# Coloquinte/sleekit

Measured on AMD Instinct MI355X. Metric: Mweights/sec quantized (GPTQ 3-bit, 4096x4096 layer), higher is better.
Workload: dtype f64; 1 GPU; 8 layers 4096x4096, 8-level uniform codebook (GPTQ 3-bit), act_order=diag, damp=0.01, local-search moves=0, layer error included; distinct_inputs=8, allocator_settle_steps=15, gpu_max_hw_queues=4

## Files before the change

sleekit_amd/csrc/api.hip:

```cpp
#include "mfma32.h"
#include "mfma64.h"

namespace slk {

__global__ __launch_bounds__(256) void k_probe_f64(double *sink, int iters) {
    double4_t c0 = {0, 0, 0, 0}, c1 = c0, c2 = c0, c3 = c0;
    const double a = 1.0 + threadIdx.x * 1e-3, b = 1.0 - threadIdx.x * 1e-3;
    for (int i = 0; i < iters; ++i) {
        c0 = __builtin_amdgcn_mfma_f64_16x16x4f64(a, b, c0, 0, 0, 0);
        c1 = __builtin_amdgcn_mfma_f64_16x16x4f64(b, a, c1, 0, 0, 0);
        c2 = __builtin_amdgcn_mfma_f64_16x16x4f64(a, a, c2, 0, 0, 0);
        c3 = __builtin_amdgcn_mfma_f64_16x16x4f64(b, b, c3, 0, 0, 0);
    }
    const double4_t s = c0 + c1 + c2 + c3;
    if (s[0] + s[1] + s[2] + s[3] == 12345.678) sink[0] = s[0];
}

template <int NACC>
__global__ __launch_bounds__(256) void k_probe_f64_n(double *sink, int iters) {
    double4_t c[NACC];
    double a[NACC], b[NACC];
#pragma unroll
    for (int i = 0; i < NACC; ++i) {
        c[i] = (double4_t){0, 0, 0, 0};
// ... 67 lines not shown
}

using namespace slk;

extern "C" {

int slk_probe_chain(double *out, int iters, int mode, slk_stream_t stream) {
    SLK_REQUIRE(out && iters > 0, "bad arguments");
    hipStream_t s = as_stream(stream);
    SLK_RUN("probe_chain", 0, 0, s, k_probe_chain<<<1, 64, 0, s>>>(out, iters, mode));
    return SLK_OK;
}

size_t slk_workspace_bytes(int R, int n) {
    if (R < 0 || n <= 0) return 0;
    const size_t ld = (size_t)slk_factor_ld(n);
    const size_t rn = (size_t)(R > 0 ? R : 1) * (size_t)n;
    size_t factor = 2 * ld * ld * sizeof(double) + 2 * (ld / 64) * sizeof(int);
    size_t loop = 2 * rn * sizeof(float) + (size_t)n * sizeof(int) + 64 * sizeof(float) + 5 * 256;
    size_t search = rn * sizeof(float) + (size_t)(R + n) * sizeof(float) + (size_t)R * ((n + 127) / 128) * sizeof(float) + 4096;
    size_t error = 6 * (rn + 128 * (size_t)n) + 6 * (size_t)n * n + 4 * (size_t)R * ((n + 127) / 128) * sizeof(float) + 8192;
    size_t prep = 64 * sizeof(float) + (size_t)n * (sizeof(double) + 1);
    search += error;
    size_t m = factor;
    if (loop > m) m = loop;
    if (search > m) m = search;
    if (error > m) m = error;
    if (prep > m) m = prep;
    return m + (1u << 16);
}

size_t slk_workspace_bytes_batch(int batch, int rows_per_layer, int n) {
    if (batch < 1 || batch > 64 || rows_per_layer < 0 || n <= 0 || (long long)batch * rows_per_layer > 0x7fffffffLL) return 0;
    return slk_workspace_bytes(batch * rows_per_layer, n) + (size_t)(batch - 1) * 6 * (size_t)n * n +
           (size_t)batch * n * (sizeof(int) + sizeof(float)) + (size_t)(batch - 1) * 64 * sizeof(float) +
           4096;
}

int slk_probe_mfma_f64(double *sink, int blocks, int iters, slk_stream_t stream) {
    SLK_REQUIRE(sink && blocks > 0 && iters > 0, "bad arguments");
    hipStream_t s = as_stream(stream);
    SLK_RUN("probe_mfma_f64", 4.0 * 2048 * 4 * iters * blocks, 0, s, k_probe_f64<<<blocks, 256, 0, s>>>(sink, iters));
    return SLK_OK;
}

int slk_probe_mfma_f64_acc(double *sink, int blocks, int iters, int nacc, slk_stream_t stream) {
    SLK_REQUIRE(sink && blocks > 0 && iters > 0 && (nacc == 1 || nacc == 2 || nacc == 4 || nacc == 8 || nacc == 16), "bad arguments");
    hipStream_t s = as_stream(stream);
    if (nacc == 1)
        SLK_RUN("probe_mfma_f64", 1.0 * 2048 * 4 * iters * blocks, 0, s, k_probe_f64_n<1><<<blocks, 256, 0, s>>>(sink, iters));
    else if (nacc == 2)
        SLK_RUN("probe_mfma_f64", 2.0 * 2048 * 4 * iters * blocks, 0, s, k_probe_f64_n<2><<<blocks, 256, 0, s>>>(sink, iters));
    else if (nacc == 4)
        SLK_RUN("probe_mfma_f64", 4.0 * 2048 * 4 * iters * blocks, 0, s, k_probe_f64_n<4><<<blocks, 256, 0, s>>>(sink, iters));
    else if (nacc == 8)
        SLK_RUN("probe_mfma_f64", 8.0 * 2048 * 4 * iters * blocks, 0, s, k_probe_f64_n<8><<<blocks, 256, 0, s>>>(sink, iters));
    else
        SLK_RUN("probe_mfma_f64", 16.0 * 2048 * 4 * iters * blocks, 0, s, k_probe_f64_n<16><<<blocks, 256, 0, s>>>(sink, iters));
    return SLK_OK;
}

int slk_probe_mfma_f32(float *sink, int blocks, int iters, slk_stream_t stream) {
    SLK_REQUIRE(sink && blocks > 0 && iters > 0, "bad arguments");
    hipStream_t s = as_stream(stream);
    SLK_RUN("probe_mfma_f32", 4.0 * 4096 * 4 * iters * blocks, 0, s, k_probe_f32<<<blocks, 256, 0, s>>>(sink, iters));
    return SLK_OK;
}

}

#include <atomic>
#include <map>
#include <mutex>
#include <string>
#include <vector>
#include <strings.h>

namespace slk {
namespace {
const char *const kOptNames[OPT_COUNT] = {
    "NO_FAST_LEAF", "NO_DEFER", "NO_WINDOW2", "WIN_DBG", "NO_REGULAR_SEARCH", "NO_FAST_SEARCH_DIV",
    "NO_ERROR_SPLITK", "ERROR_CB", "NO_SYM_ERROR", "NO_BF16_ERROR", "NO_BF16_DMA", "NO_BF16_HESSIAN",
    "ERROR_F32_BELOW", "NO_BF16_ASYM", "NO_SYM_AVERAGE", "NO_WAVE_SEARCH", "LOOKAHEAD", "WINDOW_ROWS", "PANEL_SPLIT", "ROWS_BELOW_WIDE",
    "NO_LOOP_ERROR",
};
std::atomic<int> g_opts[OPT_COUNT];
std::once_flag g_opts_once;
void opts_from_env() {
    for (int i = 0; i < OPT_COUNT; ++i) {
        const std::string name = std::string("SLK_") + kOptNames[i];
        const char *v = getenv(name.c_str());
        int val = 0;
        if (v) {
            val = atoi(v);
            if (val == 0 && v[0] != '0') val = 1;
        }
        g_opts[i].store(val, std::memory_order_relaxed);
    }
}
int opt_index(const char *name) {
    if (!name) return -1;
    if (strncasecmp(name, "SLK_", 4) == 0) name += 4;
    for (int i = 0; i < OPT_COUNT; ++i)
        if (strcasecmp(name, kOptNames[i]) == 0) return i;
    return -1;
}
std::mutex g_lds_mu;
std::map<std::pair<const void *, int>, size_t> g_lds_set;
}

int opt(Opt o) {
    std::call_once(g_opts_once, opts_from_env);
    return g_opts[o].load(std::memory_order_relaxed);
}

namespace {
std::mutex g_helper_mu;
struct HelperRec {
    Helper h;
    int made;
};
std::map<std::pair<int, hipStream_t>, HelperRec> g_helpers;
}

hipError_t helper_for(hipStream_t main, int need, Helper *out) {
    if (need > HELPER_EVENTS) return hipErrorInvalidValue;
    int device = 0;
    hipError_t e = hipGetDevice(&device);
    if (e != hipSuccess) return e;
    std::lock_guard<std::mutex> lock(g_helper_mu);
    auto it = g_helpers.find({device, main});
    if (it == g_helpers.end()) {
        HelperRec r{};
        e = hipStreamCreateWithFlags(&r.h.stream, hipStreamNonBlocking);
        if (e != hipSuccess) return e;
        e = hipStreamCreateWithFlags(&r.h.stream2, hipStreamNonBlocking);
        if (e != hipSuccess) {
            (void)hipStreamDestroy(r.h.stream);
            return e;
        }
        r.h.events = new hipEvent_t[HELPER_EVENTS]();
        r.made = 0;
        it = g_helpers.emplace(std::make_pair(device, main), r).first;
    }
    HelperRec &r = it->second;
    const int had = r.made;
    while (r.made < need) {
        e = hipEventCreateWithFlags(&r.h.events[r.made], hipEventDisableTiming);
        if (e != hipSuccess) {
            while (r.made > had) (void)hipEventDestroy(r.h.events[--r.made]);
            if (had == 0) {
                (void)hipStreamDestroy(r.h.stream);
                (void)hipStreamDestroy(r.h.stream2);
                delete[] r.h.events;
                g_helpers.erase(it);
            }
            return e;
        }
        ++r.made;
    }
    *out = r.h;
    return hipSuccess;
}

static hipError_t release_helpers() {
    std::lock_guard<std::mutex> lock(g_helper_mu);
    hipError_t first = hipSuccess;
// ... 156 lines not shown
```

sleekit_amd/csrc/common.h:

```cpp
#pragma once

#include <hip/hip_runtime.h>
#include <stddef.h>
#include <stdint.h>
#include <stdio.h>

#include "../../include/sleekit_amd.h"

namespace slk {

void set_error(const char *fmt, ...);

#define SLK_REQUIRE(cond, ...)          \
    do {                                \
        if (!(cond)) {                  \
            slk::set_error(__VA_ARGS__); \
            return SLK_E_ARG;           \
        }                               \
    } while (0)

#define SLK_HIP(call)                                                                  \
    do {                                                                               \
        hipError_t e_ = (call);                                                        \
        if (e_ != hipSuccess) {                                                        \
            slk::set_error("%s failed: %s (%s:%d)", #call, hipGetErrorString(e_), __FILE__, __LINE__); \
            return SLK_E_HIP;                                                          \
        }                                                                              \
    } while (0)

#define SLK_LAUNCH_CHECK() SLK_HIP(hipGetLastError())

struct ProfScope {
    int slot;
    hipStream_t stream;
    ProfScope(const char *name, double flops, double bytes, hipStream_t s);
    ~ProfScope();
};

void prof_next_width(long workgroups);

#define SLK_RUN(name, flops, bytes, stream, ...)                 \
    do {                                                         \
        {                                                        \
            slk::ProfScope prof_scope_(name, flops, bytes, stream); \
            __VA_ARGS__;                                         \
        }                                                        \
        SLK_LAUNCH_CHECK();                                      \
    } while (0)

#define SLK_RUN_W(name, flops, bytes, wgs, stream, ...) \
    do {                                                \
        slk::prof_next_width((long)(wgs));              \
        SLK_RUN(name, flops, bytes, stream, __VA_ARGS__); \
    } while (0)

enum Opt {
    OPT_NO_FAST_LEAF,
    OPT_NO_DEFER,
    OPT_NO_WINDOW2,
    OPT_WIN_DBG,
    OPT_NO_REGULAR_SEARCH,
    OPT_NO_FAST_SEARCH_DIV,
    OPT_NO_ERROR_SPLITK,
    OPT_ERROR_CB,
    OPT_NO_SYM_ERROR,
    OPT_NO_BF16_ERROR,
    OPT_NO_BF16_DMA,
    OPT_NO_BF16_HESSIAN,
    OPT_ERROR_F32_BELOW,
    OPT_NO_BF16_ASYM,
    OPT_NO_SYM_AVERAGE,
    OPT_NO_WAVE_SEARCH,
    OPT_LOOKAHEAD,
    OPT_WINDOW_ROWS,
    OPT_PANEL_SPLIT,
    OPT_ROWS_BELOW_WIDE,
    OPT_NO_LOOP_ERROR,
    OPT_COUNT
};
int opt(Opt o);

struct Helper {
    hipStream_t stream;
    hipStream_t stream2;
    hipEvent_t *events;
};
constexpr int HELPER_EVENTS = 512;
hipError_t helper_for(hipStream_t main, int need, Helper *out);

hipError_t lds_opt_in(const void *kernel, size_t bytes);
#define SLK_LDS_OPT_IN(kernel, bytes) SLK_HIP(slk::lds_opt_in(reinterpret_cast<const void *>(kernel), (bytes)))

struct PtrTable {
    const float *p[64];
};

constexpr int LOOP_LAYERS = 16;
struct LayerTable {
    const float *W[LOOP_LAYERS], *scale[LOOP_LAYERS];
    const long long *order[LOOP_LAYERS];
    const double *U[LOOP_LAYERS];
};
template <class T>
__device__ __forceinline__ const T *layer_base(const T *const (&column)[LOOP_LAYERS], int b, size_t stride) {
    return column[b % LOOP_LAYERS] + (size_t)(b - b % LOOP_LAYERS) * stride;
}

int row_errors_products(const float *W, const float *Q, const float *const *Hs, int batch, int rpl, int n, const int *sym_known,
                        float *row_err, float *G, void *workspace, size_t ws_bytes, slk_stream_t stream);

int loop_error_means(const float *const *Hs, int batch, int n, float *out, hipStream_t s);

static inline hipStream_t as_stream(slk_stream_t s) { return reinterpret_cast<hipStream_t>(s); }

static inline size_t align_up(size_t x, size_t a) { return (x + a - 1) / a * a; }

struct Arena {
    char *base;
    size_t size, used;
    Arena(void *p, size_t bytes) : base(static_cast<char *>(p)), size(bytes), used(0) {}
    template <class T>
    T *take(size_t count) {
        size_t off = align_up(used, 256);
        size_t end = off + count * sizeof(T);
        if (end > size || base == nullptr) return nullptr;
        used = end;
        return reinterpret_cast<T *>(base + off);
    }
};

struct Grid {
    float zero, step, top;
    const float *table;
    int n;
};

static inline Grid make_grid(int levels, double lo, double hi, const float *table = nullptr) {
    Grid g;
    g.zero = (float)lo;
    g.step = (float)((hi - lo) / (double)(levels - 1));
    g.top = (float)(levels - 1);
    g.table = table;
    g.n = levels;
    return g;
}

__device__ __forceinline__ float grid_pos(float x, const Grid g, float shift, float first, float last) {
    float t = (x - g.zero) / g.step;
    t = t + shift;
    t = rintf(t);
    return fminf(fmaxf(t, first), last);
}
__device__ __forceinline__ float grid_val(float t, const Grid g) { return t * g.step + g.zero; }
__device__ __forceinline__ float grid_value(float x, const Grid g) {
    return grid_val(grid_pos(x, g, 0.0f, 0.0f, g.top), g);
}

__device__ __forceinline__ int table_index(float x, const Grid g) {
    const float *lim = g.table + g.n;
    int lo = 0, hi = g.n - 1;
// ... 106 lines not shown
```

sleekit_amd/csrc/factor.hip:

```cpp
#include <stdlib.h>

#include "mfma64.h"

namespace slk {

constexpr int PANEL = 64;
constexpr int OUTER_SMALL = 256, OUTER_LARGE = 512;
constexpr int LOOKAHEAD_MIN_TILES = 24;

__device__ long long g_panel_cycles[16];

constexpr int TP = 66;

struct PanelSmem {
    double t[PANEL][TP];
    double x[PANEL][TP];
    double a21[PANEL][TP];
    double lb[PANEL][TP];
    double rdiag[PANEL];
    int early_count;
};

#ifndef NEWTON_STEPS
#define NEWTON_STEPS 2
// ... 314 lines not shown
            acc, ts, kprev, kprev + PANEL, [&](int k, double(&v)[8]) { load8d<true>(pa + k, v); },
            [&](int k, double(&v)[8]) { load8d<true>(pb + k, v); });
        tile64_foreach2(old, acc, [&](int r, int c, double o, double v) { pc[(size_t)r * ld + c] = o - v; });
        return;
    }
    BelowSmem &sm = *reinterpret_cast<BelowSmem *>(smem_raw);
    X += (size_t)blockIdx.z * ld * ld;
    const int lane = t & 63, wave = t >> 6;
    const bool has_prev = kprev >= 0;
    const int sr = t >> 2, sc8 = (t & 3) * 16;
    const int first = (int)blockIdx.x * per_wg, last = min(first + per_wg, tiles_below);
    double vt[16], vb[16];
    auto fetch_tile = [&](int rt) {
        const int r0 = k0 + PANEL * (rt + 1);
        const double *pt = A + (size_t)(r0 + sr) * ld + k0 + sc8;
        load8d<true>(pt, *reinterpret_cast<double(*)[8]>(&vt[0]));
        load8d<true>(pt + 8, *reinterpret_cast<double(*)[8]>(&vt[8]));
        if (has_prev) {
            const double *pl = A + (size_t)(r0 + sr) * ld + kprev + sc8;
            load8d<true>(pl, *reinterpret_cast<double(*)[8]>(&vb[0]));
            load8d<true>(pl + 8, *reinterpret_cast<double(*)[8]>(&vb[8]));
        }
    };
    {
        double vx[16], vk[16];
        const double *px = X + (size_t)(k0 + sr) * ld + k0 + sc8;
        load8d<true>(px, *reinterpret_cast<double(*)[8]>(&vx[0]));
        load8d<true>(px + 8, *reinterpret_cast<double(*)[8]>(&vx[8]));
        if (has_prev) {
            const double *pk = A + (size_t)(k0 + sr) * ld + kprev + sc8;
            load8d<true>(pk, *reinterpret_cast<double(*)[8]>(&vk[0]));
            load8d<true>(pk + 8, *reinterpret_cast<double(*)[8]>(&vk[8]));
        }
        fetch_tile(first);
#pragma unroll
        for (int e = 0; e < 16; e += 2) {
            *reinterpret_cast<double2_t *>(&sm.x[sr][sc8 + e]) = (double2_t){vx[e], vx[e + 1]};
            if (has_prev) *reinterpret_cast<double2_t *>(&sm.lk[sr][sc8 + e]) = (double2_t){vk[e], vk[e + 1]};
        }
    }
    for (int rt = first; rt < last; ++rt) {
        const int r0 = k0 + PANEL * (rt + 1);
#pragma unroll
        for (int e = 0; e < 16; e += 2) {
            *reinterpret_cast<double2_t *>(&sm.a21[sr][sc8 + e]) = (double2_t){vt[e], vt[e + 1]};
            if (has_prev) *reinterpret_cast<double2_t *>(&sm.lb[sr][sc8 + e]) = (double2_t){vb[e], vb[e + 1]};
        }
        __syncthreads();
        if (rt + 1 < last) fetch_tile(rt + 1);
        if (has_prev) {
#pragma unroll
            for (int cb = 0; cb < 4; ++cb) {
                double4_t acc = {0.0, 0.0, 0.0, 0.0};
#pragma unroll
                for (int kq = 0; kq < 4; ++kq) acc = blk_mma_abt(&sm.lb[16 * wave][16 * kq], &sm.lk[16 * cb][16 * kq], acc, 1.0, lane);
                double *cp = &sm.a21[16 * wave][16 * cb];
                double4_t o = blk_load_d(cp, lane);
#pragma unroll
                for (int r = 0; r < 4; ++r) o[r] = o[r] - acc[r];
                blk_store_d(cp, lane, o);
            }
            asm volatile("s_waitcnt lgkmcnt(0)" ::: "memory");
        }
#pragma unroll
        for (int cb = 0; cb < 4; ++cb) {
            double4_t acc = {0.0, 0.0, 0.0, 0.0};
#pragma unroll
            for (int k = 0; k < 4; ++k)
                if (k <= cb) acc = blk_mma_abt(&sm.a21[16 * wave][16 * k], &sm.x[16 * cb][16 * k], acc, 1.0, lane);
#pragma unroll
            for (int r = 0; r < 4; ++r) A[(size_t)(r0 + 16 * wave + (lane >> 4) + 4 * r) * ld + k0 + 16 * cb + (lane & 15)] = acc[r];
        }
        if (rt + 1 < last) __syncthreads();
    }
}


constexpr int INFO_HANDOFF_TIMEOUT = 0x7fffffff;
constexpr bool slk_chain_addressable(int ld) { return (size_t)ld * (size_t)ld * sizeof(double) <= 0xffffffffull; }

typedef unsigned int u32x4_t __attribute__((ext_vector_type(4)));
typedef unsigned int u32x2_t __attribute__((ext_vector_type(2)));
constexpr int AUX_SC1 = 16;

struct GBuf {
    __amdgpu_buffer_rsrc_t rs;
    __device__ __forceinline__ GBuf(const double *base, size_t bytes)
        : rs(__builtin_amdgcn_make_buffer_rsrc(const_cast<double *>(base), 0, (int)(bytes > 0xffffffffull ? 0xffffffffull : bytes), 0x00020000)) {}
    template <int AUX>
    __device__ __forceinline__ double2_t load2(unsigned elem) const {
        const u32x4_t v = __builtin_amdgcn_raw_buffer_load_b128(rs, elem * 8u, 0, AUX);
        return (double2_t){__hiloint2double((int)v[1], (int)v[0]), __hiloint2double((int)v[3], (int)v[2])};
    }
    template <int AUX>
    __device__ __forceinline__ void store2(unsigned elem, double2_t x) const {
        const u32x4_t v = {(unsigned)__double2loint(x[0]), (unsigned)__double2hiint(x[0]), (unsigned)__double2loint(x[1]), (unsigned)__double2hiint(x[1])};
        __builtin_amdgcn_raw_buffer_store_b128(v, rs, elem * 8u, 0, AUX);
    }
};

__device__ __forceinline__ int flag_peek(const int *p) { return __hip_atomic_load(p, __ATOMIC_RELAXED, __HIP_MEMORY_SCOPE_AGENT); }
__device__ __forceinline__ bool flag_wait(const int *p, int want) {
    bool ok = flag_peek(p) >= want;
    if (!ok) {
        const unsigned long long t0 = __builtin_amdgcn_s_memrealtime();
        for (;;) {
            __builtin_amdgcn_s_sleep(1);
            if (flag_peek(p) >= want) {
                ok = true;
                break;
            }
            if (__builtin_amdgcn_s_memrealtime() - t0 > 200000000ull) break;
        }
    }
    __builtin_amdgcn_fence(__ATOMIC_ACQUIRE, "wavefront");
    return ok;
}
__device__ __forceinline__ void flag_publish(int *p, int value) {
    asm volatile("s_waitcnt vmcnt(0)" ::: "memory");
    __syncthreads();
    if (threadIdx.x == 0) __hip_atomic_store(p, value, __ATOMIC_RELAXED, __HIP_MEMORY_SCOPE_AGENT);
}

struct TileRegs {
    double2_t v[8];
};
template <int AUX, int J0 = 0, int J1 = 8>
__device__ __forceinline__ void tile_fetch(TileRegs &r, const GBuf &g, unsigned elem0, int ld) {
    const int t = threadIdx.x;
#pragma unroll
    for (int j = J0; j < J1; ++j) r.v[j] = g.load2<AUX>(elem0 + (unsigned)(8 * j + (t >> 5)) * (unsigned)ld + 2u * (t & 31));
}
template <int J0 = 0, int J1 = 8>
__device__ __forceinline__ void tile_stash(double (*img)[TP], const TileRegs &r) {
    const int t = threadIdx.x;
#pragma unroll
    for (int j = J0; j < J1; ++j) *reinterpret_cast<double2_t *>(&img[8 * j + (t >> 5)][2 * (t & 31)]) = r.v[j];
}
template <int AUX, int J0 = 0, int J1 = 8>
__device__ __forceinline__ void tile_store_from_lds(const GBuf &g, unsigned elem0, int ld, const double (*img)[TP]) {
    const int t = threadIdx.x;
#pragma unroll
    for (int j = J0; j < J1; ++j)
        g.store2<AUX>(elem0 + (unsigned)(8 * j + (t >> 5)) * (unsigned)ld + 2u * (t & 31), *reinterpret_cast<const double2_t *>(&img[8 * j + (t >> 5)][2 * (t & 31)]));
}

template <class Early>
__device__ __forceinline__ int diag_tile_factor(PanelSmem &sm, int lane, int wave, Early rows_0_and_1_are_in) {
    auto diag_inverse = [&](int kb) {
        const int c0 = 16 * kb, c = lane & 15;
        double xv[16];
#pragma unroll
        for (int i = 0; i < 16; ++i) {
            double s = 0.0;
#pragma unroll
            for (int u = 0; u < i; ++u) s = __builtin_fma(sm.t[c0 + i][c0 + u], xv[u], s);
            xv[i] = ((c == i ? 1.0 : 0.0) - s) * sm.rdiag[c0 + i];
        }
        if (lane < 16) {
#pragma unroll
            for (int i = 0; i < 16; ++i) sm.x[c0 + i][c0 + c] = xv[i];
        }
    };
    auto block_owner = [](int rb, int cb) { return cb == 1 ? rb : (rb == 3 && cb == 2 ? 2 : 1); };
    auto block_update = [&](int rb, int cb, int kb) {
        double *c = &sm.t[16 * rb][16 * cb];
        blk_store_d(c, lane, blk_mma_abt(&sm.t[16 * rb][16 * kb], &sm.t[16 * cb][16 * kb], blk_load_d(c, lane), -1.0, lane));
    };
    auto x_inner = [&](int rb, int cb) {
        double4_t sacc = {0.0, 0.0, 0.0, 0.0};
#pragma unroll
        for (int k = 0; k < 4; ++k)
            if (k >= cb && k < rb) sacc = blk_mma_ab(&sm.t[16 * rb][16 * k], &sm.x[16 * k][16 * cb], sacc, lane);
        return sacc;
    };
    auto x_finish = [&](int rb, int cb, double4_t sacc) {
        const double4_t z = {0.0, 0.0, 0.0, 0.0};
        blk_store_d(&sm.x[16 * rb][16 * cb], lane, blk_mma_a_reg(&sm.x[16 * rb][16 * rb], sacc, z, -1.0, lane));
    };
    auto x_block = [&](int rb, int cb) { x_finish(rb, cb, x_inner(rb, cb)); };
    auto own_writes = [&]() { asm volatile("s_waitcnt lgkmcnt(0)" ::: "memory"); };
    int first_bad = PANEL;
#pragma unroll
    for (int kb = 0; kb < 4; ++kb) {
        const int c0 = 16 * kb;
        if (wave == 0) {
            const int row = c0 + lane;
            const bool live = row < PANEL;
            double a[16];
#pragma unroll
            for (int c = 0; c < 16; ++c) a[c] = live ? sm.t[live ? row : 0][c0 + c] : 0.0;
#pragma unroll
            for (int j = 0; j < 16; ++j) {
                double piv = readlane_f64(a[j], j);
                const bool bad = !(piv > 0.0);
                first_bad = (bad && first_bad == PANEL) ? c0 + j : first_bad;
                piv = bad ? 1.0 : piv;
                const double r = rsqrt_newton(piv);
                const double lj = a[j] * r;
                a[j] = lj;
                sm.rdiag[c0 + j] = r;
#pragma unroll
                for (int c = j + 1; c < 16; ++c) a[c] = __builtin_fma(-lj, readlane_f64(lj, c), a[c]);
            }
            if (live) {
#pragma unroll
                for (int c = 0; c < 16; ++c) sm.t[row][c0 + c] = (c0 + c <= row) ? a[c] : 0.0;
            }
        } else if (kb == 0) {
        } else if (wave == 3) {
            diag_inverse(kb - 1);
            own_writes();
            if (kb == 2) x_block(1, 0);
            if (kb == 3) {
                x_block(2, 1);
                x_block(2, 0);
            }
        } else {
#pragma unroll
            for (int rb = kb + 1; rb < 4; ++rb)
#pragma unroll
                for (int cb = kb + 1; cb <= rb; ++cb)
                    if (block_owner(rb, cb) == wave) block_update(rb, cb, kb - 1);
            if (kb == 3) rows_0_and_1_are_in(wave - 1);
        }
        __syncthreads();
        if (kb < 3) {
#pragma unroll
            for (int rb = kb + 1; rb < 4; ++rb)
                if (block_owner(rb, kb + 1) == wave) block_update(rb, kb + 1, kb);
            __syncthreads();
        }
    }
    double4_t row3 = {0.0, 0.0, 0.0, 0.0};
    if (wave == 3) diag_inverse(3);
    else row3 = x_inner(3, wave);
    __syncthreads();
    if (wave < 3) x_finish(3, wave, row3);
    __syncthreads();
    return first_bad;
}

template <bool BELOW>
__global__ __launch_bounds__(256) void k_chol_chain(double *__restrict__ Aall, int ld, int K0, int nb, double *__restrict__ Xall,
                                                    int *__restrict__ info, int *__restrict__ flags_all, int dbg) {
    extern __shared__ __attribute__((aligned(16))) char smem_raw[];
    PanelSmem &sm = *reinterpret_cast<PanelSmem *>(smem_raw);
    const int t = threadIdx.x, lane = t & 63, wave = t >> 6;
    const int r = BELOW ? nb + (int)blockIdx.x : (int)blockIdx.x, nt = ld / PANEL, p0 = K0 / PANEL;
    const int rq = BELOW ? nb : r;
    const size_t mat = (size_t)ld * ld;
    double *A = Aall + (size_t)blockIdx.z * mat;
    const GBuf ga(A, mat * sizeof(double)), gx(Xall + (size_t)blockIdx.z * mat, mat * sizeof(double));
    info += blockIdx.z;
    int *xready = flags_all + (size_t)blockIdx.z * 2 * nt, *rowdone = xready + nt;
    const int row0 = K0 + PANEL * r;
    auto elem = [&](int tr, int tc) { return (unsigned)(K0 + PANEL * tr) * (unsigned)ld + (unsigned)(K0 + PANEL * tc); };
    bool alive = true;
    if (t == 0) sm.early_count = 0;
    const bool timing = !BELOW && dbg && r > 0 && blockIdx.z == 0 && wave == 0;
    long long tmark = 0;
    auto lap = [&](int slot) {
        if (timing) {
            const long long now = (long long)__builtin_readcyclecounter();
            if (lane == 0 && slot >= 0) atomicAdd(reinterpret_cast<unsigned long long *>(&g_panel_cycles[slot]), (unsigned long long)(now - tmark));
            tmark = now;
        }
    };

    double4_t tp[3];
    if constexpr (!BELOW) {
        int i = 0;
#pragma unroll
        for (int rb = 0; rb < 4; ++rb)
#pragma unroll
            for (int cb = 0; cb <= rb; ++cb, ++i)
                if ((i & 3) == wave) {
#pragma unroll
                    for (int j = 0; j < 4; ++j) {
                        const int rr = 16 * rb + (lane >> 4) + 4 * j, cc = 16 * cb + (lane & 15);
                        tp[i >> 2][j] = (r > 0 || cc <= rr) ? A[(size_t)(row0 + rr) * ld + row0 + cc] : 0.0;
                    }
                }
    }
    auto update_cn = [&](double4_t(&cn)[4]) {
#pragma unroll
        for (int cb = 0; cb < 4; ++cb) {
            double4_t acc = {0.0, 0.0, 0.0, 0.0};
#pragma unroll
            for (int kq = 0; kq < 4; ++kq) acc = blk_mma_abt(&sm.lb[16 * wave][16 * kq], &sm.t[16 * cb][16 * kq], acc, 1.0, lane);
#pragma unroll
            for (int j = 0; j < 4; ++j) cn[cb][j] = cn[cb][j] - acc[j];
        }
    };

    auto row_done = [&](int count) {
        if constexpr (BELOW) {
            asm volatile("s_waitcnt vmcnt(0)" ::: "memory");
            __syncthreads();
        } else {
            flag_publish(&rowdone[p0 + r], count);
        }
    };
    if (rq > 0) {
        TileRegs ra, rb_;
        double4_t cn[4];
        tile_fetch<0>(ra, ga, elem(r, 0), ld);
        tile_stash(sm.a21, ra);
        for (int q = 0; q < rq; ++q) {
            const bool more = q + 1 < rq;
            if (more) {
#pragma unroll
                for (int cb = 0; cb < 4; ++cb)
#pragma unroll
                    for (int j = 0; j < 4; ++j)
                        cn[cb][j] = A[(size_t)(row0 + 16 * wave + (lane >> 4) + 4 * j) * ld + K0 + PANEL * (q + 1) + 16 * cb + (lane & 15)];
                if (q > 0) {
                    if (!BELOW) alive = alive && flag_wait(&rowdone[p0 + q + 1], 1);
                    tile_fetch<AUX_SC1>(ra, ga, elem(r, 0), ld);
                    tile_fetch<AUX_SC1>(rb_, ga, elem(q + 1, 0), ld);
                }
                for (int s = 0; s < q; ++s) {
                    __syncthreads();
                    tile_stash(sm.lb, ra);
                    tile_stash(sm.t, rb_);
                    __syncthreads();
                    if (s + 1 < q) {
                        if (!BELOW && alive) alive = flag_wait(&rowdone[p0 + q + 1], s + 2);
                        tile_fetch<AUX_SC1>(ra, ga, elem(r, s + 1), ld);
                        tile_fetch<AUX_SC1>(rb_, ga, elem(q + 1, s + 1), ld);
                    }
                    update_cn(cn);
                }
            }
            const bool last = !BELOW && q + 1 == r;
            auto l_block = [&](int cb) {
                double4_t acc = {0.0, 0.0, 0.0, 0.0};
#pragma unroll
                for (int k = 0; k < 4; ++k)
                    if (k <= cb) acc = blk_mma_abt(&sm.a21[16 * wave][16 * k], &sm.x[16 * cb][16 * k], acc, 1.0, lane);
                blk_store_d(&sm.lb[16 * wave][16 * cb], lane, acc);
            };
            double4_t tacc[3];
            auto t_terms = [&](int kq0, int kq1) {
                int i = 0;
#pragma unroll
                for (int rb = 0; rb < 4; ++rb)
#pragma unroll
                    for (int cb = 0; cb <= rb; ++cb, ++i)
                        if ((i & 3) == wave) {
                            double4_t acc = kq0 == 0 ? (double4_t){0.0, 0.0, 0.0, 0.0} : tacc[i >> 2];
#pragma unroll
                            for (int kq = 0; kq < 4; ++kq)
                                if (kq >= kq0 && kq < kq1) acc = blk_mma_abt(&sm.lb[16 * rb][16 * kq], &sm.lb[16 * cb][16 * kq], acc, 1.0, lane);
                            tacc[i >> 2] = acc;
                        }
            };
            if (!BELOW && alive) alive = flag_wait(&xready[p0 + q], 1);
            tile_fetch<AUX_SC1, 0, 4>(ra, gx, elem(q, q), ld);
            __syncthreads();
            tile_stash<0, 4>(sm.x, ra);
            __syncthreads();
            l_block(0);
            l_block(1);
            __syncthreads();
            if (!BELOW) t_terms(0, 2);
            if (!BELOW && alive) alive = flag_wait(&xready[p0 + q], 2);
            if (last) lap(-1);
            tile_fetch<AUX_SC1, 4, 8>(ra, gx, elem(q, q), ld);
            tile_stash<4, 8>(sm.x, ra);
            __syncthreads();
            if (last) lap(0);
            l_block(2);
            l_block(3);
            __syncthreads();
            if (last) lap(1);
            tile_store_from_lds<AUX_SC1>(ga, elem(r, q), ld, sm.lb);
            if constexpr (!BELOW) {
                t_terms(2, 4);
                int i = 0;
#pragma unroll
                for (int rb = 0; rb < 4; ++rb)
#pragma unroll
                    for (int cb = 0; cb <= rb; ++cb, ++i)
                        if ((i & 3) == wave) {
#pragma unroll
                            for (int j = 0; j < 4; ++j) tp[i >> 2][j] = tp[i >> 2][j] - tacc[i >> 2][j];
                            if (last) blk_store_d(&sm.t[16 * rb][16 * cb], lane, tp[i >> 2]);
                        }
            }
            if (more) {
                if (!BELOW && alive) alive = flag_wait(&rowdone[p0 + q + 1], q + 1);
                tile_fetch<AUX_SC1>(rb_, ga, elem(q + 1, q), ld);
                tile_stash(sm.t, rb_);
                row_done(q + 1);
                update_cn(cn);
#pragma unroll
                for (int cb = 0; cb < 4; ++cb) blk_store_d(&sm.a21[16 * wave][16 * cb], lane, cn[cb]);
            } else {
                lap(2);
                row_done(q + 1);
                lap(3);
            }
        }
    } else if (!BELOW) {
        int i = 0;
#pragma unroll
        for (int rb = 0; rb < 4; ++rb)
#pragma unroll
            for (int cb = 0; cb <= rb; ++cb, ++i)
                if ((i & 3) == wave) blk_store_d(&sm.t[16 * rb][16 * cb], lane, tp[i >> 2]);
        for (int e = t; e < PANEL * PANEL; e += 256) sm.x[e >> 6][e & 63] = 0.0;
        __syncthreads();
    }
    if constexpr (BELOW) return;
    lap(4);
    const int first_bad = diag_tile_factor(sm, lane, wave, [&](int rowblock) {
#pragma unroll
        for (int j = 0; j < 8; ++j) {
            const int row = 16 * rowblock + 2 * j + (lane >> 5);
            gx.store2<AUX_SC1>(elem(r, r) + (unsigned)row * (unsigned)ld + 2u * (lane & 31), *reinterpret_cast<const double2_t *>(&sm.x[row][2 * (lane & 31)]));
        }
        asm volatile("s_waitcnt vmcnt(0)" ::: "memory");
        int arrived = 0;
        if (lane == 0) arrived = __hip_atomic_fetch_add(&sm.early_count, 1, __ATOMIC_RELAXED, __HIP_MEMORY_SCOPE_WORKGROUP);
        arrived = __builtin_amdgcn_readfirstlane(arrived);
        if (arrived == 1) {
            if (lane == 0) __hip_atomic_store(&xready[p0 + r], 1, __ATOMIC_RELAXED, __HIP_MEMORY_SCOPE_AGENT);
            asm volatile("s_waitcnt vmcnt(0)" ::: "memory");
        }
    });
    lap(5);
    if (t == 0) {
        int expect = 0;
        if (!alive) {
            __hip_atomic_store(info, INFO_HANDOFF_TIMEOUT, __ATOMIC_RELAXED, __HIP_MEMORY_SCOPE_AGENT);
        } else if (first_bad != PANEL) {
            __hip_atomic_compare_exchange_strong(info, &expect, row0 + first_bad + 1, __ATOMIC_RELAXED, __ATOMIC_RELAXED, __HIP_MEMORY_SCOPE_AGENT);
        }
    }
    tile_store_from_lds<AUX_SC1, 4, 8>(gx, elem(r, r), ld, sm.x);
    flag_publish(&xready[p0 + r], 2);
    lap(6);
    if (timing && lane == 0) atomicAdd(reinterpret_cast<unsigned long long *>(&g_panel_cycles[15]), 1ull);
}

struct RowsBelowSmem {
    double own[8][16][TP];
    double bt[PANEL][TP];
    double c[16][TP];
};
__global__ __launch_bounds__(256) void k_chol_rows_below(double *__restrict__ Aall, int ld, int K0, int nb, const double *__restrict__ Xall) {
    extern __shared__ __attribute__((aligned(16))) char smem_raw[];
    RowsBelowSmem &sm = *reinterpret_cast<RowsBelowSmem *>(smem_raw);
    const int t = threadIdx.x, lane = t & 63, wave = t >> 6;
    const size_t mat = (size_t)ld * ld;
    double *A = Aall + (size_t)blockIdx.z * mat;
    const GBuf ga(A, mat * sizeof(double)), gx(Xall + (size_t)blockIdx.z * mat, mat * sizeof(double));
    const int rows0 = K0 + PANEL * nb + 16 * blockIdx.x;
    auto tile_elem = [&](int tr, int tc) { return (unsigned)(K0 + PANEL * tr) * (unsigned)ld + (unsigned)(K0 + PANEL * tc); };
    auto load_c = [&](int q) {
        const double *p = A + (size_t)(rows0 + (lane >> 4)) * ld + K0 + PANEL * q + 16 * wave + (lane & 15);
        return (double4_t){p[0], p[(size_t)4 * ld], p[(size_t)8 * ld], p[(size_t)12 * ld]};
    };
    TileRegs nx;
    tile_fetch<0>(nx, gx, tile_elem(0, 0), ld);
    double4_t c = load_c(0), cnext = load_c(nb > 1 ? 1 : 0);
    for (int q = 0; q < nb; ++q) {
        for (int s = 0; s <= q; ++s) {
            const bool tri = s == q;
            __syncthreads();
            tile_stash(sm.bt, nx);
            if (tri) blk_store_d(&sm.c[0][16 * wave], lane, c);
            __syncthreads();
            if (!tri) {
                if (s + 1 < q) tile_fetch<0>(nx, ga, tile_elem(q, s + 1), ld);
                else tile_fetch<0>(nx, gx, tile_elem(q, q), ld);
            } else if (q + 1 < nb) {
                tile_fetch<0>(nx, ga, tile_elem(q + 1, 0), ld);
            }
            if (!tri) {
                double4_t acc = {0.0, 0.0, 0.0, 0.0};
#pragma unroll
                for (int kq = 0; kq < 4; ++kq) acc = blk_mma_abt(&sm.own[s][0][16 * kq], &sm.bt[16 * wave][16 * kq], acc, 1.0, lane);
                c = c - acc;
            } else {
                double4_t acc = {0.0, 0.0, 0.0, 0.0};
#pragma unroll
                for (int k = 0; k < 4; ++k)
                    if (k <= wave) acc = blk_mma_abt(&sm.c[0][16 * k], &sm.bt[16 * wave][16 * k], acc, 1.0, lane);
#pragma unroll
                for (int j = 0; j < 4; ++j) A[(size_t)(rows0 + (lane >> 4) + 4 * j) * ld + K0 + PANEL * q + 16 * wave + (lane & 15)] = acc[j];
                blk_store_d(&sm.own[q][0][16 * wave], lane, acc);
                c = cnext;
                if (q + 2 < nb) cnext = load_c(q + 2);
            }
        }
    }
}

__global__ __launch_bounds__(256) void k_syrk_tiles(double *__restrict__ A, int ld, int ti0, int tj0, int ka,
                                                    int kb) {
    __shared__ __attribute__((aligned(16))) Tile64Smem sm;
    A += (size_t)blockIdx.z * ld * ld;
    const int bi = ti0 + blockIdx.y, bj = tj0 + blockIdx.x;
    if (bj > bi) return;
    Acc64 acc;
    acc.zero();
    const int t = threadIdx.x;
    const double *pa = A + ((size_t)bi * TILE + (t >> 2)) * ld + (t & 3) * 8;
    const double *pb = A + ((size_t)bj * TILE + (t >> 2)) * ld + (t & 3) * 8;
    double *pc = A + (size_t)bi * TILE * ld + (size_t)bj * TILE;
    Acc64 old;
    tile64_map(old, [&](int r, int c) { return pc[(size_t)r * ld + c]; });
    tile64_mac<false>(
        acc, sm, ka, kb, [&](int k0, double(&v)[8]) { load8d<true>(pa + k0, v); },
        [&](int k0, double(&v)[8]) { load8d<true>(pb + k0, v); });
    tile64_foreach2(old, acc, [&](int r, int c, double o, double v) { pc[(size_t)r * ld + c] = o - v; });
}

__global__ __launch_bounds__(256) void k_syrk_triangle(double *__restrict__ A, int ld, int t0, int m, int ka, int kb) {
    __shared__ __attribute__((aligned(16))) Tile64Smem sm;
    A += (size_t)blockIdx.z * ld * ld;
    const int total = m * (m + 1) / 2, per_xcd = (total + 7) / 8;
    const int lin = (blockIdx.x & 7) * per_xcd + (blockIdx.x >> 3);
    if (lin >= total) return;
    int row = (int)((sqrtf(8.0f * (float)lin + 1.0f) - 1.0f) * 0.5f);
// ... 20 lines not shown
    __shared__ __attribute__((aligned(16))) Tile64Smem sm;
    L += (size_t)blockIdx.z * ld * ld;
    X += (size_t)blockIdx.z * ld * ld;
    S += (size_t)blockIdx.z * ld * ld;
    const int id = blockIdx.x;
    const int per_node = s * s, node = node0 + id / per_node, in_node = id % per_node;
    const int deep = in_node / s, other = in_node % s;
    const int lo = node * 2 * s, mid = lo + s;
    const int bi = (STAGE == 0) ? mid + other : mid + (s - 1 - deep);
    const int bj = (STAGE == 0) ? lo + deep : lo + other;
    if (bi >= nt) return;
    Acc64 acc;
    acc.zero();
    const int t = threadIdx.x;
    if (STAGE == 0) {
        const double *pa = L + ((size_t)bi * TILE + (t >> 2)) * ld + (t & 3) * 8;
        const double *pb = X + (size_t)(t >> 3) * ld + (size_t)bj * TILE + (t & 7) * 2;
        tile64_mac<true>(
            acc, sm, bj * TILE, mid * TILE, [&](int k0, double(&v)[8]) { load8d<true>(pa + k0, v); },
            [&](int k0, double(&v)[8]) { load8d_cols(pb + (size_t)k0 * ld, v); });
        double *pc = S + (size_t)bi * TILE * ld + (size_t)bj * TILE;
        tile64_foreach(acc, [&](int r, int c, double v) { pc[(size_t)r * ld + c] = v; });
    } else {
        const double *pa = X + ((size_t)bi * TILE + (t >> 2)) * ld + (t & 3) * 8;
        const double *pb = S + (size_t)(t >> 3) * ld + (size_t)bj * TILE + (t & 7) * 2;
        tile64_mac<true>(
            acc, sm, mid * TILE, (bi + 1) * TILE, [&](int k0, double(&v)[8]) { load8d<true>(pa + k0, v); },
            [&](int k0, double(&v)[8]) { load8d_cols(pb + (size_t)k0 * ld, v); });
        double *pc = X + (size_t)bi * TILE * ld + (size_t)bj * TILE;
        tile64_foreach(acc, [&](int r, int c, double v) { pc[(size_t)r * ld + c] = -v; });
    }
}

__global__ __launch_bounds__(256) void k_flip_out(const double *__restrict__ X, int ld, int n,
                                                  double *__restrict__ U) {
    X += (size_t)blockIdx.z * ld * ld;
    U += (size_t)blockIdx.z * n * n;
    for (int i = blockIdx.x; i < n; i += gridDim.x) {
        const double *src = X + (size_t)(n - 1 - i) * ld;
        double *dst = U + (size_t)i * n;
        for (int j = threadIdx.x; j < n; j += blockDim.x) dst[j] = (j >= i) ? src[n - 1 - j] : 0.0;
    }
}

__global__ void k_clear_info(int *info, int *flags, int per_matrix) {
    if (threadIdx.x == 0) info[blockIdx.x] = 0;
    if (flags)
        for (int i = threadIdx.x; i < per_matrix; i += blockDim.x) flags[(size_t)blockIdx.x * per_matrix + i] = 0;
}

}

using namespace slk;

static int chol_inverse_impl(double *A, int batch, int n, double *U, int *info, void *workspace, size_t ws_bytes,
                             slk_stream_t stream, bool want_lookahead) {
    const int ld = slk_factor_ld(n);
    const int nt = ld / TILE;
    const unsigned B = (unsigned)batch;
    const double Bd = (double)batch;
    Arena ws(workspace, ws_bytes);
    double *X = ws.take<double>((size_t)ld * ld * batch);
    double *S = ws.take<double>((size_t)ld * ld * batch);
    int *flags = ws.take<int>((size_t)batch * 2 * nt);
    if (!X || !S || !flags) {
        set_error("workspace too small for %d factorisation(s) of %d x %d", batch, n, n);
        return SLK_E_WS;
    }
    hipStream_t s = as_stream(stream);
    const int OUTER = n >= 4096 ? OUTER_LARGE : OUTER_SMALL;
    SLK_LDS_OPT_IN(k_chol_panel, sizeof(PanelSmem));
    SLK_RUN_W("clear_info", 0, 4, 1, s, k_clear_info<<<B, 64, 0, s>>>(info, flags, 2 * nt));

    Helper helper{};
    const bool lookahead = (want_lookahead || opt(OPT_LOOKAHEAD)) && nt >= LOOKAHEAD_MIN_TILES + OUTER / TILE && nt / (OUTER / TILE) < HELPER_EVENTS / 3;
    if (lookahead) SLK_HIP(helper_for(s, 3 * (nt / (OUTER / TILE) + 1), &helper));
    const int sp = opt(OPT_PANEL_SPLIT);
    const bool chain = (sp == 0 || sp == 3) && slk_chain_addressable(ld);
    const bool split = !chain && !want_lookahead && sp != 2 && (sp == 1 || batch > 1 || n >= 8192);
    if (split) SLK_LDS_OPT_IN(k_panel_below, sizeof(BelowSmem));
    if (chain) {
        SLK_LDS_OPT_IN(k_chol_chain<false>, sizeof(PanelSmem));
        SLK_LDS_OPT_IN(k_chol_chain<true>, sizeof(PanelSmem));
        SLK_LDS_OPT_IN(k_chol_rows_below, sizeof(RowsBelowSmem));
    }
    int inv_done[2][16] = {{0}, {0}};
    auto inverse_nodes = [&](int tiles_done, hipStream_t st) -> int {
        int li = 0;
        for (int lvl = 1; lvl < nt; lvl *= 2, ++li) {
            const int all = (nt + 2 * lvl - 1) / (2 * lvl);
            for (int stage = 0; stage < 2; ++stage) {
                int ready;
                if (tiles_done >= nt) ready = all;
                else if (stage == 0) ready = tiles_done >= lvl ? (tiles_done - lvl) / (2 * lvl) + 1 : 0;
                else ready = tiles_done / (2 * lvl);
                if (ready > all) ready = all;
                const int first = inv_done[stage][li], count = ready - first;
                if (count <= 0) continue;
                inv_done[stage][li] = ready;
                double fl = 0, tiles = 0;
                for (int nd = first; nd < ready; ++nd) {
                    const int lo = nd * 2 * lvl, mid = lo + lvl, hi = lo + 2 * lvl < nt ? lo + 2 * lvl : nt;
                    for (int bi = mid; bi < hi; ++bi)
                        for (int bj = lo; bj < mid; ++bj) {
                            fl += 2.0 * 64 * 64 * 64 * (stage == 0 ? mid - bj : bi + 1 - mid);
                            tiles += 1;
                        }
                }
                if (tiles == 0) continue;
                dim3 grid(count * lvl * lvl, 1, B);
                if (stage == 0)
                    SLK_RUN_W("trtri_stage0", Bd * fl, Bd * (fl / 64 * 8.0 / 2 + tiles * 8.0 * 64 * 64), tiles * batch, st,
                              k_trtri_level<0><<<grid, 256, 0, st>>>(A, X, S, ld, nt, lvl, first));
                else
                    SLK_RUN_W("trtri_stage1", Bd * fl, Bd * (fl / 64 * 8.0 / 2 + tiles * 8.0 * 64 * 64), tiles * batch, st,
                              k_trtri_level<1><<<grid, 256, 0, st>>>(A, X, S, ld, nt, lvl, first));
            }
        }
        return SLK_OK;
    };
    const int EV = chain ? 3 : 2;
    int block = 0, forked = -1;
    int inverse_on_helper = -1;
    for (int K0 = 0; K0 < ld; K0 += OUTER) {
        const int K1 = K0 + OUTER < ld ? K0 + OUTER : ld;
        if (chain) {
            const int nb = (K1 - K0) / PANEL, below_tiles = (ld - K1) / PANEL;
            const double e = 64.0 * nb;
            SLK_RUN_W("chol_chain", Bd * e * e * e / 3.0, Bd * 12.0 * e * e, nb * batch, s,
                      k_chol_chain<false><<<dim3(nb, 1, B), 256, sizeof(PanelSmem), s>>>(A, ld, K0, nb, X, info, flags, opt(OPT_WIN_DBG) & 8));
            if (below_tiles > 0 && forked >= 0) {
                SLK_HIP(hipStreamWaitEvent(s, helper.events[EV * forked + 1], 0));
                forked = -1;
            }
            const int rw = opt(OPT_ROWS_BELOW_WIDE);
            const bool wide = rw == 1 || (rw == 0 && 4 * below_tiles * batch >= 1024);
            if (below_tiles > 0 && wide)
                SLK_RUN_W("chol_rows_below", Bd * 64.0 * below_tiles * e * e, Bd * (16.0 * 64 * below_tiles * e + 4.0 * e * e), below_tiles * batch, s,
                          k_chol_chain<true><<<dim3(below_tiles, 1, B), 256, sizeof(PanelSmem), s>>>(A, ld, K0, nb, X, info, flags, 0));
            else if (below_tiles > 0)
                SLK_RUN_W("chol_rows_below", Bd * 64.0 * below_tiles * e * e, Bd * (16.0 * 64 * below_tiles * e + 4.0 * e * e), 4 * below_tiles * batch, s,
                          k_chol_rows_below<<<dim3(4 * below_tiles, 1, B), 256, sizeof(RowsBelowSmem), s>>>(A, ld, K0, nb, X));
        }
        for (int k0 = K0; k0 < K1 && !chain; k0 += PANEL) {
            const int below = (ld - k0) / PANEL;
            const int kprev = k0 > K0 ? k0 - PANEL : -1;
            const int rest_cols = kprev >= 0 ? (K1 - k0) / PANEL - 1 : 0;
            int rest = 0;
            for (int c = 0; c < rest_cols; ++c) rest += nt - (k0 / TILE + 1 + c);
            const double prologue = kprev >= 0 ? (double)below * 2.0 * 64 * 64 * 64 + (double)below * 2.0 * 64 * 64 * 64 : 0.0;
            if (split) {
                const double pro1 = kprev >= 0 ? 2.0 * 64 * 64 * 64 : 0.0;
                SLK_RUN_W("chol_panel", Bd * (2.0 / 3.0 * 64 * 64 * 64 + pro1), Bd * 16.0 * 64 * 64, batch, s,
                          k_chol_panel<<<dim3(1, 1, B), 256, sizeof(PanelSmem), s>>>(A, ld, k0, kprev, 1, 0, X, info, opt(OPT_WIN_DBG) & 8));
                if (below - 1 + rest > 0) {
                    const int per_wg = 2;
                    const int nbw = (below - 1 + per_wg - 1) / per_wg;
                    SLK_RUN_W("chol_panel_below",
                              Bd * ((double)(below - 1) * 64 * 64 * 64 + (kprev >= 0 ? (double)(below - 1) * 2.0 * 64 * 64 * 64 : 0.0) +
                                    (double)rest * 2.0 * 64 * 64 * PANEL),
                              Bd * (24.0 * (below - 1) * 64 * 64 + (double)rest * 16.0 * 64 * 64), (nbw + rest) * batch, s,
                              k_panel_below<<<dim3(nbw + rest, 1, B), 256, sizeof(BelowSmem), s>>>(A, ld, k0, kprev, nbw, rest_cols, X, below - 1,
                                                                                                  per_wg));
                }
            } else {
                SLK_RUN_W("chol_panel",
                          Bd * (2.0 / 3.0 * 64 * 64 * 64 + (double)(below - 1) * 64 * 64 * 64 + prologue + (double)rest * 2.0 * 64 * 64 * PANEL),
                          Bd * (16.0 * below * 64 * 64 + (double)rest * 16.0 * 64 * 64), (below + rest) * batch, s,
                          k_chol_panel<<<dim3(below + rest, 1, B), 256, sizeof(PanelSmem), s>>>(A, ld, k0, kprev, below, rest_cols, X, info,
                                                                                                opt(OPT_WIN_DBG) & 8));
            }
        }
        const int t0 = K1 / TILE;
        if (nt > t0) {
            const int m = nt - t0, total = m * (m + 1) / 2;
            const double tiles = total;
            const int ahead = OUTER / TILE;
            if (lookahead && chain && m >= LOOKAHEAD_MIN_TILES) {
                SLK_HIP(hipEventRecord(helper.events[EV * block], s));
                const int nbn = ahead < m ? ahead : m, td = nbn * (nbn + 1) / 2;
                SLK_RUN_W("chol_syrk_ahead", Bd * td * 2.0 * 64 * 64 * (K1 - K0), Bd * (16.0 * nbn * 64 * (K1 - K0) + td * 16.0 * 64 * 64), td * batch, s,
                          k_syrk_tiles<<<dim3(nbn, nbn, B), 256, 0, s>>>(A, ld, t0, t0, K0, K1));
                SLK_HIP(hipStreamWaitEvent(helper.stream, helper.events[EV * block], 0));
                const int m2 = m - nbn, total2 = m2 * (m2 + 1) / 2;
                if (m2 > 0) {
                    SLK_RUN_W("chol_syrk_outer", Bd * (double)nbn * m2 * 2.0 * 64 * 64 * (K1 - K0), Bd * (8.0 * (ld - K1) * (K1 - K0) + (double)nbn * m2 * 16.0 * 64 * 64),
                              (double)nbn * m2 * batch, helper.stream,
                              k_syrk_tiles<<<dim3(nbn, m2, B), 256, 0, helper.stream>>>(A, ld, t0 + nbn, t0, K0, K1));
                    SLK_RUN_W("chol_syrk_outer", Bd * total2 * 2.0 * 64 * 64 * (K1 - K0), Bd * (8.0 * (ld - K1) * (K1 - K0) + total2 * 16.0 * 64 * 64),
                              (double)total2 * batch, helper.stream,
                              k_syrk_triangle<<<dim3(8 * ((total2 + 7) / 8), 1, B), 256, 0, helper.stream>>>(A, ld, t0 + nbn, m2, K0, K1));
                }
                SLK_HIP(hipEventRecord(helper.events[EV * block + 1], helper.stream));
                forked = block;
                SLK_HIP(hipStreamWaitEvent(helper.stream2, helper.events[EV * block], 0));
                {
                    const int rc = inverse_nodes(t0, helper.stream2);
                    if (rc != SLK_OK) return rc;
                }
                SLK_HIP(hipEventRecord(helper.events[EV * block + 2], helper.stream2));
                inverse_on_helper = block;
            } else if (lookahead && m >= LOOKAHEAD_MIN_TILES) {
                if (block > 0) SLK_HIP(hipStreamWaitEvent(s, helper.events[2 * (block - 1) + 1], 0));
                SLK_HIP(hipEventRecord(helper.events[2 * block], s));
                const double ta = (double)ahead * m - 6;
                SLK_RUN_W("chol_syrk_ahead", Bd * ta * 2.0 * 64 * 64 * (K1 - K0), Bd * (8.0 * (ld - K1) * (K1 - K0) + ta * 16.0 * 64 * 64),
                          ta * batch, s, k_syrk_tiles<<<dim3(ahead, m, B), 256, 0, s>>>(A, ld, t0, t0, K0, K1));
                SLK_HIP(hipStreamWaitEvent(helper.stream, helper.events[2 * block], 0));
                const int m2 = m - ahead, total2 = m2 * (m2 + 1) / 2;
                SLK_RUN_W("chol_syrk_outer", Bd * total2 * 2.0 * 64 * 64 * (K1 - K0), Bd * (8.0 * (ld - K1) * (K1 - K0) + total2 * 16.0 * 64 * 64),
                          (double)total2 * batch, helper.stream,
                          k_syrk_triangle<<<dim3(8 * ((total2 + 7) / 8), 1, B), 256, 0, helper.stream>>>(A, ld, t0 + ahead, m2, K0, K1));
                SLK_HIP(hipEventRecord(helper.events[2 * block + 1], helper.stream));
// ... 67 lines not shown
```

Measured before the change: 6374 Mweights/s.

## Fuse below-panel row updates into the Cholesky chain kernel launch

Adds a combined kernel where extra blocks beyond the chain's diagonal panels process the rows below the outer block. These blocks wait on the chain's per-row flags instead of launching a separate kernel after the chain finishes. It is enabled by default when the total block count is small (at most 80) and lookahead is off, so it applies only to the small trailing outer blocks in this 4096 case. This removes a kernel launch and the serialization between the two kernels, at the cost of spin-waiting blocks and a possible timeout path.

```diff
diff --git a/sleekit_amd/csrc/api.hip b/sleekit_amd/csrc/api.hip
--- a/sleekit_amd/csrc/api.hip
+++ b/sleekit_amd/csrc/api.hip
@@ -173,7 +173,7 @@
     "NO_FAST_LEAF", "NO_DEFER", "NO_WINDOW2", "WIN_DBG", "NO_REGULAR_SEARCH", "NO_FAST_SEARCH_DIV",
     "NO_ERROR_SPLITK", "ERROR_CB", "NO_SYM_ERROR", "NO_BF16_ERROR", "NO_BF16_DMA", "NO_BF16_HESSIAN",
     "ERROR_F32_BELOW", "NO_BF16_ASYM", "NO_SYM_AVERAGE", "NO_WAVE_SEARCH", "LOOKAHEAD", "WINDOW_ROWS", "PANEL_SPLIT", "ROWS_BELOW_WIDE",
-    "NO_LOOP_ERROR",
+    "NO_LOOP_ERROR", "CHAIN_CARRIES_BELOW",
 };
 std::atomic<int> g_opts[OPT_COUNT];
 std::once_flag g_opts_once;
diff --git a/sleekit_amd/csrc/common.h b/sleekit_amd/csrc/common.h
--- a/sleekit_amd/csrc/common.h
+++ b/sleekit_amd/csrc/common.h
@@ -76,6 +76,7 @@
     OPT_PANEL_SPLIT,
     OPT_ROWS_BELOW_WIDE,
     OPT_NO_LOOP_ERROR,
+    OPT_CHAIN_CARRIES_BELOW,
     OPT_COUNT
 };
 int opt(Opt o);
diff --git a/sleekit_amd/csrc/factor.hip b/sleekit_amd/csrc/factor.hip
--- a/sleekit_amd/csrc/factor.hip
+++ b/sleekit_amd/csrc/factor.hip
@@ -420,6 +420,8 @@
 typedef unsigned int u32x4_t __attribute__((ext_vector_type(4)));
 typedef unsigned int u32x2_t __attribute__((ext_vector_type(2)));
 constexpr int AUX_SC1 = 16;
+constexpr int CHAIN_CARRY_CAP = 80;
+constexpr bool CHAIN_CARRY_BY_RULE = true;
 
 struct GBuf {
     __amdgpu_buffer_rsrc_t rs;
@@ -579,13 +581,14 @@
     return first_bad;
 }
 
-template <bool BELOW>
-__global__ __launch_bounds__(256) void k_chol_chain(double *__restrict__ Aall, int ld, int K0, int nb, double *__restrict__ Xall,
-                                                    int *__restrict__ info, int *__restrict__ flags_all, int dbg) {
-    extern __shared__ __attribute__((aligned(16))) char smem_raw[];
-    PanelSmem &sm = *reinterpret_cast<PanelSmem *>(smem_raw);
+enum ChainForm { CHAIN_ROWS, BELOW_ROWS, CHAIN_AND_BELOW };
+template <int FORM>
+__device__ __forceinline__ void chol_chain_walk(PanelSmem &sm, double *__restrict__ Aall, int ld, int K0, int nb, double *__restrict__ Xall,
+                                                int *__restrict__ info, int *__restrict__ flags_all, int dbg) {
+    const bool BELOW = FORM == BELOW_ROWS || (FORM == CHAIN_AND_BELOW && (int)blockIdx.x >= nb);
+    constexpr bool WAITS = FORM != BELOW_ROWS;
     const int t = threadIdx.x, lane = t & 63, wave = t >> 6;
-    const int r = BELOW ? nb + (int)blockIdx.x : (int)blockIdx.x, nt = ld / PANEL, p0 = K0 / PANEL;
+    const int r = FORM == BELOW_ROWS ? nb + (int)blockIdx.x : (int)blockIdx.x, nt = ld / PANEL, p0 = K0 / PANEL;
     const int rq = BELOW ? nb : r;
     const size_t mat = (size_t)ld * ld;
     double *A = Aall + (size_t)blockIdx.z * mat;
@@ -607,7 +610,7 @@
     };
 
     double4_t tp[3];
-    if constexpr (!BELOW) {
+    if (!BELOW) {
         int i = 0;
 #pragma unroll
         for (int rb = 0; rb < 4; ++rb)
@@ -633,7 +636,7 @@
     };
 
     auto row_done = [&](int count) {
-        if constexpr (BELOW) {
+        if (BELOW) {
             asm volatile("s_waitcnt vmcnt(0)" ::: "memory");
             __syncthreads();
         } else {
@@ -654,7 +657,7 @@
                     for (int j = 0; j < 4; ++j)
                         cn[cb][j] = A[(size_t)(row0 + 16 * wave + (lane >> 4) + 4 * j) * ld + K0 + PANEL * (q + 1) + 16 * cb + (lane & 15)];
                 if (q > 0) {
-                    if (!BELOW) alive = alive && flag_wait(&rowdone[p0 + q + 1], 1);
+                    if (WAITS) alive = alive && flag_wait(&rowdone[p0 + q + 1], 1);
                     tile_fetch<AUX_SC1>(ra, ga, elem(r, 0), ld);
                     tile_fetch<AUX_SC1>(rb_, ga, elem(q + 1, 0), ld);
                 }
@@ -664,7 +667,7 @@
                     tile_stash(sm.t, rb_);
                     __syncthreads();
                     if (s + 1 < q) {
-                        if (!BELOW && alive) alive = flag_wait(&rowdone[p0 + q + 1], s + 2);
+                        if (WAITS && alive) alive = flag_wait(&rowdone[p0 + q + 1], s + 2);
                         tile_fetch<AUX_SC1>(ra, ga, elem(r, s + 1), ld);
                         tile_fetch<AUX_SC1>(rb_, ga, elem(q + 1, s + 1), ld);
                     }
@@ -694,7 +697,7 @@
                             tacc[i >> 2] = acc;
                         }
             };
-            if (!BELOW && alive) alive = flag_wait(&xready[p0 + q], 1);
+            if (WAITS && alive) alive = flag_wait(&xready[p0 + q], 1);
             tile_fetch<AUX_SC1, 0, 4>(ra, gx, elem(q, q), ld);
             __syncthreads();
             tile_stash<0, 4>(sm.x, ra);
@@ -703,7 +706,7 @@
             l_block(1);
             __syncthreads();
             if (!BELOW) t_terms(0, 2);
-            if (!BELOW && alive) alive = flag_wait(&xready[p0 + q], 2);
+            if (WAITS && alive) alive = flag_wait(&xready[p0 + q], 2);
             if (last) lap(-1);
             tile_fetch<AUX_SC1, 4, 8>(ra, gx, elem(q, q), ld);
             tile_stash<4, 8>(sm.x, ra);
@@ -714,7 +717,7 @@
             __syncthreads();
             if (last) lap(1);
             tile_store_from_lds<AUX_SC1>(ga, elem(r, q), ld, sm.lb);
-            if constexpr (!BELOW) {
+            if (!BELOW) {
                 t_terms(2, 4);
                 int i = 0;
 #pragma unroll
@@ -728,7 +731,7 @@
                         }
             }
             if (more) {
-                if (!BELOW && alive) alive = flag_wait(&rowdone[p0 + q + 1], q + 1);
+                if (WAITS && alive) alive = flag_wait(&rowdone[p0 + q + 1], q + 1);
                 tile_fetch<AUX_SC1>(rb_, ga, elem(q + 1, q), ld);
                 tile_stash(sm.t, rb_);
                 row_done(q + 1);
@@ -751,7 +754,10 @@
         for (int e = t; e < PANEL * PANEL; e += 256) sm.x[e >> 6][e & 63] = 0.0;
         __syncthreads();
     }
-    if constexpr (BELOW) return;
+    if (BELOW) {
+        if (WAITS && !alive && t == 0) __hip_atomic_store(info, INFO_HANDOFF_TIMEOUT, __ATOMIC_RELAXED, __HIP_MEMORY_SCOPE_AGENT);
+        return;
+    }
     lap(4);
     const int first_bad = diag_tile_factor(sm, lane, wave, [&](int rowblock) {
 #pragma unroll
@@ -781,6 +787,18 @@
     flag_publish(&xready[p0 + r], 2);
     lap(6);
     if (timing && lane == 0) atomicAdd(reinterpret_cast<unsigned long long *>(&g_panel_cycles[15]), 1ull);
+}
+
+template <bool BELOW>
+__global__ __launch_bounds__(256) void k_chol_chain(double *__restrict__ Aall, int ld, int K0, int nb, double *__restrict__ Xall,
+                                                    int *__restrict__ info, int *__restrict__ flags_all, int dbg) {
+    extern __shared__ __attribute__((aligned(16))) char smem_raw[];
+    chol_chain_walk<BELOW ? BELOW_ROWS : CHAIN_ROWS>(*reinterpret_cast<PanelSmem *>(smem_raw), Aall, ld, K0, nb, Xall, info, flags_all, dbg);
+}
+__global__ __launch_bounds__(256) void k_chol_chain_below(double *__restrict__ Aall, int ld, int K0, int nb, double *__restrict__ Xall,
+                                                          int *__restrict__ info, int *__restrict__ flags_all, int dbg) {
+    extern __shared__ __attribute__((aligned(16))) char smem_raw[];
+    chol_chain_walk<CHAIN_AND_BELOW>(*reinterpret_cast<PanelSmem *>(smem_raw), Aall, ld, K0, nb, Xall, info, flags_all, dbg);
 }
 
 struct RowsBelowSmem {
@@ -967,6 +985,7 @@
     if (chain) {
         SLK_LDS_OPT_IN(k_chol_chain<false>, sizeof(PanelSmem));
         SLK_LDS_OPT_IN(k_chol_chain<true>, sizeof(PanelSmem));
+        SLK_LDS_OPT_IN(k_chol_chain_below, sizeof(PanelSmem));
         SLK_LDS_OPT_IN(k_chol_rows_below, sizeof(RowsBelowSmem));
     }
     int inv_done[2][16] = {{0}, {0}};
@@ -1010,10 +1029,20 @@
     for (int K0 = 0; K0 < ld; K0 += OUTER) {
         const int K1 = K0 + OUTER < ld ? K0 + OUTER : ld;
         if (chain) {
-            const int nb = (K1 - K0) / PANEL, below_tiles = (ld - K1) / PANEL;
+            const int nb = (K1 - K0) / PANEL;
+            int below_tiles = (ld - K1) / PANEL;
             const double e = 64.0 * nb;
-            SLK_RUN_W("chol_chain", Bd * e * e * e / 3.0, Bd * 12.0 * e * e, nb * batch, s,
-                      k_chol_chain<false><<<dim3(nb, 1, B), 256, sizeof(PanelSmem), s>>>(A, ld, K0, nb, X, info, flags, opt(OPT_WIN_DBG) & 8));
+            const int cc = opt(OPT_CHAIN_CARRIES_BELOW);
+            const bool carry = below_tiles > 0 && !lookahead && opt(OPT_ROWS_BELOW_WIDE) == 0 && (nb + below_tiles) * batch <= CHAIN_CARRY_CAP &&
+                               (cc == 1 || (cc == 0 && CHAIN_CARRY_BY_RULE));
+            if (carry) {
+                SLK_RUN_W("chol_chain", Bd * (e * e * e / 3.0 + 64.0 * below_tiles * e * e), Bd * (12.0 * e * e + 16.0 * 64 * below_tiles * e + 4.0 * e * e),
+                          (nb + below_tiles) * batch, s,
+                          k_chol_chain_below<<<dim3(nb + below_tiles, 1, B), 256, sizeof(PanelSmem), s>>>(A, ld, K0, nb, X, info, flags, opt(OPT_WIN_DBG) & 8));
+                below_tiles = 0;
+            } else
+                SLK_RUN_W("chol_chain", Bd * e * e * e / 3.0, Bd * 12.0 * e * e, nb * batch, s,
+                          k_chol_chain<false><<<dim3(nb, 1, B), 256, sizeof(PanelSmem), s>>>(A, ld, K0, nb, X, info, flags, opt(OPT_WIN_DBG) & 8));
             if (below_tiles > 0 && forked >= 0) {
                 SLK_HIP(hipStreamWaitEvent(s, helper.events[EV * forked + 1], 0));
                 forked = -1;
```

Result: faster. 6544 Mweights/s, median of 6 (+2.7%).
